# wavey-ai/soundkit

Hardware: AMD Instinct MI355X
Metric: AAC-LC 1024-sample frames/s (whole node) + xrealtime, batch=4096 48 kHz stereo (higher is better)
Workload: dtype f32 (synthesis f32; s16 between the kernels as in the reference; FIR: the 16-bit samples as 2 x f16 exactly, the f32 taps as 2 x f16 to 2^-24, f32 accumulate; 1.0e-7 rel. RMS vs f64)

## Files before the change

soundkit_amd/csrc/aac_synth.hip:

```cpp
#include "sk_device.h"

#define SK_SYNTH_LOAD(p) (*(p))
#define SK_SYNTH_STORE(v, p) (*(p) = (v))

namespace sk {

namespace {

typedef float f2 __attribute__((ext_vector_type(2)));
typedef float f4 __attribute__((ext_vector_type(4)));

#ifndef SK_SYNTH_BLOCK_WAVES
#define SK_SYNTH_BLOCK_WAVES 4
#endif
constexpr int kWavesPerBlock = SK_SYNTH_BLOCK_WAVES;
#ifndef SK_WAVES_PER_SIMD
#define SK_WAVES_PER_SIMD 3
#endif
#ifndef SK_PREFETCH_DEPTH
#define SK_PREFETCH_DEPTH 1
#endif
constexpr int kDepth = SK_PREFETCH_DEPTH;
constexpr int kWavesPerSimd = SK_WAVES_PER_SIMD;
constexpr int kExchange = 576;
// ... 495 lines not shown
    wave_sync();
    f2 o[16], d[16];
#pragma unroll
    for (int half = 0; half < 2; ++half) {
#pragma unroll
        for (int r = 0; r < 8; ++r) *reinterpret_cast<lds_f4 *>(stage + 2 * lane + 128 * r) = (f4){0.f, 0.f, 0.f, 0.f};
        wave_sync();
#pragma unroll
        for (int parity = 0; parity < 2; ++parity) {
#pragma unroll
            for (int w = parity; w < 8; w += 2)
#pragma unroll
                for (int m = 0; m < 4; ++m) {
                    const int base = 448 + 128 * w + 64 * m;
                    if ((base >> 10) != half) continue;
                    lds_f2 *at = stage + (base & 1023) + lane;
                    *at = *at + smp[w][m];
                }
            wave_sync();
        }
        if (half == 0) read_positions2(stage, lane, o);
        else read_positions2(stage, lane, d);
        wave_sync();
    }
    f2 pcm[16];
#pragma unroll
    for (int i = 0; i < 16; ++i) pcm[i] = o[i] + dly[i];
    write_positions2((lds_f2 *)ex, lane, pcm);
    write_positions2(stage, lane, d);
    wave_sync();
}

template <bool OUT16, bool WITH_SHORT>
__global__ __launch_bounds__(kWavesPerBlock * 64, 2) void k_aac_synth_pair(SynthArgs a) {
    constexpr bool LDS_WIN = !WITH_SHORT;
    __shared__ f4 lds[kWavesPerBlock][kPairExchange];
    __shared__ f4 win_tab[LDS_WIN ? 2048 : 1];
    __shared__ f2 stage_lds[WITH_SHORT ? kWavesPerBlock : 1][WITH_SHORT ? kStage : 2];
    __shared__ f2 tw_tab[512];
    __shared__ f2 t64_tab[64];
    __shared__ float short_win_tab[WITH_SHORT ? 512 : 2];
    __shared__ f2 short_tw_tab[WITH_SHORT ? 128 : 1];

    const int lane = threadIdx.x & 63;
    const int wave = __builtin_amdgcn_readfirstlane(threadIdx.x >> 6);
    for (int i = threadIdx.x; i < 512; i += kWavesPerBlock * 64) tw_tab[i] = reinterpret_cast<const f2 *>(a.t.tw_long)[i];
    if (threadIdx.x < 64) t64_tab[threadIdx.x] = reinterpret_cast<const f2 *>(a.t.w64)[((threadIdx.x >> 3) * (threadIdx.x & 7)) & 63];
    if (WITH_SHORT) {
        for (int i = threadIdx.x; i < 512; i += kWavesPerBlock * 64) short_win_tab[i] = a.t.win[4096 + i];
        if (threadIdx.x < 128)
            short_tw_tab[threadIdx.x] = threadIdx.x < 64 ? reinterpret_cast<const f2 *>(a.t.w64)[threadIdx.x] : reinterpret_cast<const f2 *>(a.t.tw_short)[threadIdx.x - 64];
    }
    if (LDS_WIN)
        for (int i = threadIdx.x; i < 2048; i += kWavesPerBlock * 64) win_tab[i] = reinterpret_cast<const f4 *>(a.t.win)[i < 1024 ? i : i + 128];
    __syncthreads();
    const lds_f *win_lds = (const lds_f *)win_tab;

    const uint32_t pair_id = blockIdx.x * kWavesPerBlock + wave;
    if (2 * pair_id + 1 >= a.n_tasks) return;
    lds_f4 *ex = (lds_f4 *)lds[wave];
    const lds_f2 *tw_lds = (const lds_f2 *)tw_tab;
    const lds_f2 *t64 = (const lds_f2 *)t64_tab;

    const SynthTask task_a = a.tasks[2 * pair_id], task_b = a.tasks[2 * pair_id + 1];
    const uint32_t count = __builtin_amdgcn_readfirstlane(task_a.count);
    if (count == 0) return;
    const uint32_t state_a = __builtin_amdgcn_readfirstlane(task_a.state), state_b = __builtin_amdgcn_readfirstlane(task_b.state);
    const const_entries ent_a = as_constant(a.entries + __builtin_amdgcn_readfirstlane(task_a.begin));
    const const_entries ent_b = as_constant(a.entries + __builtin_amdgcn_readfirstlane(task_b.begin));

    const int hi3 = lane >> 3, lo3 = lane & 7;
    const f2 base2 = reinterpret_cast<const f2 *>(a.t.w512)[hi3 * lo3];

    float *delay_a = a.delay + (size_t)state_a * 1024, *delay_b = a.delay + (size_t)state_b * 1024;
    int prev_a = __builtin_amdgcn_readfirstlane((int)a.prev_shape[state_a]);
    int prev_b = __builtin_amdgcn_readfirstlane((int)a.prev_shape[state_b]);
    float dly_a[16], dly_b[16];
    auto load_state = [&](const float *p, float (&d)[16]) {
#pragma unroll
        for (int r = 0; r < 2; ++r) {
            const int j = 4 * lane + 256 * r;
            const f4 f = *reinterpret_cast<const f4 *>(p + j);
            const f4 m = *reinterpret_cast<const f4 *>(p + 1020 - j);
            d[8 * r + 0] = f.x; d[8 * r + 1] = f.y; d[8 * r + 2] = f.z; d[8 * r + 3] = f.w;
            d[8 * r + 4] = m.x; d[8 * r + 5] = m.y; d[8 * r + 6] = m.z; d[8 * r + 7] = m.w;
        }
    };
    load_state(delay_a, dly_a);
    load_state(delay_b, dly_b);

    auto load_spectrum = [&](f2 (&xin)[8], const_entries entries, uint32_t e) {
        const float *src = a.coeffs + (size_t)__builtin_amdgcn_readfirstlane(entries[e].off1024) * 1024 + 2 * lane;
#pragma unroll
        for (int r = 0; r < 8; ++r) xin[r] = SK_SYNTH_LOAD(reinterpret_cast<const f2 *>(src + 128 * r));
    };
    struct Win {
        f4 w1f[2], w1m[2], w2f[2], w2m[2];
    };
    auto load_windows = [&](Win &w, int seq, int prev_shape, int shape) {
        const float *w1 = first_half_window(a.t.win, seq, prev_shape);
        const float *w2 = second_half_window(a.t.win, seq, shape);
#pragma unroll
        for (int r = 0; r < 2; ++r) {
            const int j = 4 * lane + 256 * r;
            w.w1f[r] = *reinterpret_cast<const f4 *>(w1 + j);
            w.w1m[r] = *reinterpret_cast<const f4 *>(w1 + 1020 - j);
            w.w2f[r] = *reinterpret_cast<const f4 *>(w2 + j);
            w.w2m[r] = *reinterpret_cast<const f4 *>(w2 + 1020 - j);
        }
    };
    auto emit = [&](int r, f2 F0, f2 F1, f2 M0, f2 M1, const Win &w, int w1_at, int w2_at, float (&dly)[16], float *out_ptr, int16_t *out16_ptr) {
        const int j = 4 * lane + 256 * r;
        f4 W1f, W1m, W2f, W2m;
        if constexpr (LDS_WIN) {
            W1f = *reinterpret_cast<const lds_f4 *>(win_lds + w1_at + j), W1m = *reinterpret_cast<const lds_f4 *>(win_lds + w1_at + 1020 - j);
            W2f = *reinterpret_cast<const lds_f4 *>(win_lds + w2_at + j), W2m = *reinterpret_cast<const lds_f4 *>(win_lds + w2_at + 1020 - j);
        } else {
            W1f = w.w1f[r], W1m = w.w1m[r], W2f = w.w2f[r], W2m = w.w2m[r];
        }
        f4 f, m;
        f.x = -F0.x * W1f.x + dly[8 * r + 0]; f.y = -M1.y * W1f.y + dly[8 * r + 1];
        f.z = -F1.x * W1f.z + dly[8 * r + 2]; f.w = -M0.y * W1f.w + dly[8 * r + 3];
        m.x = M0.y * W1m.x + dly[8 * r + 4]; m.y = F1.x * W1m.y + dly[8 * r + 5];
        m.z = M1.y * W1m.z + dly[8 * r + 6]; m.w = F0.x * W1m.w + dly[8 * r + 7];
        if (OUT16) {
            SK_SYNTH_STORE(pack4_s16(f), reinterpret_cast<u2 *>(out16_ptr + j));
            SK_SYNTH_STORE(pack4_s16(m), reinterpret_cast<u2 *>(out16_ptr + 1020 - j));
        } else {
            SK_SYNTH_STORE(f, reinterpret_cast<f4 *>(out_ptr + j));
            SK_SYNTH_STORE(m, reinterpret_cast<f4 *>(out_ptr + 1020 - j));
        }
        dly[8 * r + 0] = F0.y * W2f.x; dly[8 * r + 1] = M1.x * W2f.y;
        dly[8 * r + 2] = F1.y * W2f.z; dly[8 * r + 3] = M0.x * W2f.w;
        dly[8 * r + 4] = M0.x * W2m.x; dly[8 * r + 5] = F1.y * W2m.y;
        dly[8 * r + 6] = M1.x * W2m.z; dly[8 * r + 7] = F0.y * W2m.w;
    };

    lds_f2 *stage = (lds_f2 *)stage_lds[WITH_SHORT ? wave : 0];
    auto store_pcm = [&](const float (&pcm)[16], uint32_t off) __attribute__((always_inline)) {
#pragma unroll
        for (int r = 0; r < 2; ++r) {
            const int j = 4 * lane + 256 * r;
            const f4 f = (f4){pcm[8 * r + 0], pcm[8 * r + 1], pcm[8 * r + 2], pcm[8 * r + 3]};
            const f4 m = (f4){pcm[8 * r + 4], pcm[8 * r + 5], pcm[8 * r + 6], pcm[8 * r + 7]};
            if (OUT16) {
                SK_SYNTH_STORE(pack4_s16(f), reinterpret_cast<u2 *>(a.pcm16 + (size_t)off * 1024 + j));
                SK_SYNTH_STORE(pack4_s16(m), reinterpret_cast<u2 *>(a.pcm16 + (size_t)off * 1024 + 1020 - j));
            } else {
                SK_SYNTH_STORE(f, reinterpret_cast<f4 *>(a.pcm + (size_t)off * 1024 + j));
                SK_SYNTH_STORE(m, reinterpret_cast<f4 *>(a.pcm + (size_t)off * 1024 + 1020 - j));
            }
        }
    };

    f2 xa[8], xb[8];
    load_spectrum(xa, ent_a, 0);
    load_spectrum(xb, ent_b, 0);
    for (uint32_t e = 0; e < count; ++e) {
        const uint32_t off_a = __builtin_amdgcn_readfirstlane(ent_a[e].off1024), off_b = __builtin_amdgcn_readfirstlane(ent_b[e].off1024);
        const uint32_t win_a = __builtin_amdgcn_readfirstlane(ent_a[e].win), win_b = __builtin_amdgcn_readfirstlane(ent_b[e].win);
        const int shape_a = (win_a >> 2) & 1, shape_b = (win_b >> 2) & 1;
        if constexpr (WITH_SHORT) {
            if ((win_a & 3u) == 2u) {
// ... 51 lines not shown
            const f2 tx = splat(t.x), ty = splat(t.y);
            z[r] = {odd * ty - even * tx, odd * tx + even * ty};
        }
        Win wa, wb;
        int w1_a = 0, w2_a = 0, w1_b = 0, w2_b = 0;
        if constexpr (LDS_WIN) {
            const int seq_a = (int)(win_a & 3), seq_b = (int)(win_b & 3);
            w1_a = seq_a == 3 ? 6144 + 1024 * prev_a : 2048 * prev_a, w2_a = seq_a == 1 ? 4096 + 1024 * shape_a : 2048 * shape_a + 1024;
            w1_b = seq_b == 3 ? 6144 + 1024 * prev_b : 2048 * prev_b, w2_b = seq_b == 1 ? 4096 + 1024 * shape_b : 2048 * shape_b + 1024;
        } else {
            load_windows(wa, (int)(win_a & 3), prev_a, shape_a);
            load_windows(wb, (int)(win_b & 3), prev_b, shape_b);
        }
        {
            const uint32_t ahead = e + 1 < count ? e + 1 : count - 1;
            load_spectrum(xa, ent_a, ahead);
            load_spectrum(xb, ent_b, ahead);
        }
        fft512(z, ex, t64, base2, lane);
#pragma unroll
        for (int j = 0; j < 8; ++j) {
            const f2 t = tw_lds[lane + 64 * j];
            const f2 tx = splat(t.x), ty = splat(t.y);
            const c2 v = {fma2(tx, z[j].re, -(ty * -z[j].im)), fma2(tx, -z[j].im, ty * z[j].re)};
            ex[lane + 64 * j] = as_slot(v);
        }
        wave_sync();
        float *out_a = OUT16 ? nullptr : a.pcm + (size_t)off_a * 1024, *out_b = OUT16 ? nullptr : a.pcm + (size_t)off_b * 1024;
        int16_t *out16_a = OUT16 ? a.pcm16 + (size_t)off_a * 1024 : nullptr, *out16_b = OUT16 ? a.pcm16 + (size_t)off_b * 1024 : nullptr;
#pragma unroll
        for (int r = 0; r < 2; ++r) {
            const int q = 2 * lane + 128 * r;
            const f4 F0 = ex[256 + q], F1 = ex[257 + q], M0 = ex[254 - q], M1 = ex[255 - q];
            emit(r, (f2){F0.x, F0.z}, (f2){F1.x, F1.z}, (f2){M0.x, M0.z}, (f2){M1.x, M1.z}, wa, w1_a, w2_a, dly_a, out_a, out16_a);
            emit(r, (f2){F0.y, F0.w}, (f2){F1.y, F1.w}, (f2){M0.y, M0.w}, (f2){M1.y, M1.w}, wb, w1_b, w2_b, dly_b, out_b, out16_b);
        }
        wave_sync();
        prev_a = shape_a;
        prev_b = shape_b;
    }
    auto store_state = [&](float *p, const float (&d)[16]) {
#pragma unroll
        for (int r = 0; r < 2; ++r) {
            const int j = 4 * lane + 256 * r;
            *reinterpret_cast<f4 *>(p + j) = (f4){d[8 * r + 0], d[8 * r + 1], d[8 * r + 2], d[8 * r + 3]};
            *reinterpret_cast<f4 *>(p + 1020 - j) = (f4){d[8 * r + 4], d[8 * r + 5], d[8 * r + 6], d[8 * r + 7]};
        }
    };
    store_state(delay_a, dly_a);
    store_state(delay_b, dly_b);
    if (lane == 0) {
        a.prev_shape[state_a] = (uint8_t)prev_a;
        a.prev_shape[state_b] = (uint8_t)prev_b;
    }
}

constexpr int kTailRing = 2048;
constexpr int kTailDepth = 2;

__global__ __launch_bounds__(128, 2) void k_aac_tail(TailArgs ta) {
    const SynthArgs &a = ta.s;
    __shared__ f2 lds[2][kExchange];
    __shared__ f2 tw_tab[512];
    __shared__ f2 t64_tab[64];
    __shared__ __attribute__((aligned(16))) uint16_t ring_lds[2][2][kTailRing];
    __shared__ __attribute__((aligned(16))) uint32_t xchg[2][2][128];

    const int lane = threadIdx.x & 63;
    const int wave = __builtin_amdgcn_readfirstlane((int)(threadIdx.x >> 6));
    for (int i = threadIdx.x; i < 512; i += 128) tw_tab[i] = reinterpret_cast<const f2 *>(a.t.tw_long)[i];
    if (threadIdx.x < 64) t64_tab[threadIdx.x] = reinterpret_cast<const f2 *>(a.t.w64)[((threadIdx.x >> 3) * (threadIdx.x & 7)) & 63];
    for (int i = threadIdx.x; i < 2 * 2 * kTailRing / 8; i += 128) reinterpret_cast<sk_u32x4 *>(&ring_lds[0][0][0])[i] = (sk_u32x4){0u, 0u, 0u, 0u};
    __syncthreads();

    const uint32_t pair_id = blockIdx.x;
    lds_f2 *ex = (lds_f2 *)lds[wave];
    const lds_f2 *tw_lds = (const lds_f2 *)tw_tab;
    const lds_f2 *t64 = (const lds_f2 *)t64_tab;
    unsigned char *ring = reinterpret_cast<unsigned char *>(&ring_lds[wave][0][0]);

    const SynthTask task_v = a.tasks[2 * pair_id + (uint32_t)wave];
// ... 226 lines not shown
}

}

hipError_t launch_zero_spans(float *base, const uint32_t *ids, uint32_t n, uint32_t span_floats, hipStream_t s) {
    if (n == 0) return hipSuccess;
    if (span_floats % 4) return hipErrorInvalidValue;
    hipLaunchKernelGGL(k_zero_spans, dim3(n), dim3(256), 0, s, base, ids, span_floats);
    return hipGetLastError();
}

hipError_t launch_reset_streams(float *delay, uint8_t *shape, uint32_t *pns, const uint32_t *ids, uint32_t n, hipStream_t s) {
    if (n == 0) return hipSuccess;
    hipLaunchKernelGGL(k_reset_streams, dim3(n), dim3(256), 0, s, delay, shape, pns, ids);
    return hipGetLastError();
}

hipError_t launch_aac_synth(const SynthArgs &a, hipStream_t s) {
    if (a.n_tasks == 0) return hipSuccess;
    const uint32_t blocks = (a.n_tasks + kWavesPerBlock - 1) / kWavesPerBlock;
    if (a.only_long) {
        if (a.pcm16) hipLaunchKernelGGL((k_aac_synth<true, true>), dim3(blocks), dim3(kWavesPerBlock * 64), 0, s, a);
        else hipLaunchKernelGGL((k_aac_synth<false, true>), dim3(blocks), dim3(kWavesPerBlock * 64), 0, s, a);
    } else {
        if (a.pcm16) hipLaunchKernelGGL((k_aac_synth<true, false>), dim3(blocks), dim3(kWavesPerBlock * 64), 0, s, a);
        else hipLaunchKernelGGL((k_aac_synth<false, false>), dim3(blocks), dim3(kWavesPerBlock * 64), 0, s, a);
    }
    return hipGetLastError();
}

hipError_t launch_aac_synth_pairs(const SynthArgs &a, bool with_short, hipStream_t s) {
    if (a.n_tasks < 2) return hipSuccess;
    if (a.n_tasks & 1) return hipErrorInvalidValue;
    const uint32_t pairs = a.n_tasks / 2, blocks = (pairs + kWavesPerBlock - 1) / kWavesPerBlock;
    const dim3 grid(blocks), block(kWavesPerBlock * 64);
    if (with_short) {
        if (a.pcm16) hipLaunchKernelGGL((k_aac_synth_pair<true, true>), grid, block, 0, s, a);
        else hipLaunchKernelGGL((k_aac_synth_pair<false, true>), grid, block, 0, s, a);
    } else {
        if (a.pcm16) hipLaunchKernelGGL((k_aac_synth_pair<true, false>), grid, block, 0, s, a);
        else hipLaunchKernelGGL((k_aac_synth_pair<false, false>), grid, block, 0, s, a);
    }
    return hipGetLastError();
}

hipError_t launch_aac_tail(const TailArgs &ta, hipStream_t s) {
    if (ta.s.n_tasks < 2) return hipSuccess;
    if ((ta.s.n_tasks & 1) || !ta.afrag_f16 || !ta.out16 || ta.stream_stride == 0) return hipErrorInvalidValue;
    hipLaunchKernelGGL(k_aac_tail, dim3(ta.s.n_tasks / 2), dim3(128), 0, s, ta);
    return hipGetLastError();
}

hipError_t launch_frames_to_s16(const float *planar, int16_t *out, const FrameSpan *frames, uint32_t n, hipStream_t s) {
    if (n == 0) return hipSuccess;
    hipLaunchKernelGGL(k_frames_to_s16, dim3(n), dim3(256), 0, s, planar, out, frames, n);
    return hipGetLastError();
}

hipError_t launch_dequantize(const int16_t *q, const int16_t *sf, float *out, size_t n, const float *pow43,
                             const float *sftab, hipStream_t s) {
    if (n == 0) return hipSuccess;
    size_t blocks = (n + 255) / 256;
    if (blocks > 8192) blocks = 8192;
    hipLaunchKernelGGL(k_dequantize, dim3((unsigned)blocks), dim3(256), 0, s, q, sf, out, n, pow43, sftab);
    return hipGetLastError();
}

}
// ... 1 lines not shown
```

soundkit_amd/csrc/engine.cpp:

```cpp
#include "../../include/soundkit_amd.h"
#include "sk_abi.h"

#include <hip/hip_runtime.h>

#include <cmath>
#include <cstdio>
#include <chrono>
#include <cstdlib>
#include <cstring>
#include <algorithm>
#include <atomic>
#include <thread>
#include <map>
#include <mutex>
#include <new>
#include <string>
#include <unordered_map>
#include <vector>

#include "aac_entropy_tables.h"
#include "sk_device.h"

namespace {

// ... 136 lines not shown
        y[x] = val;
    }
    sum /= (float)factor;
    for (size_t p = 0; p < npoints; ++p) taps[p] = y[factor * p + (factor - 1)] / sum;
}

void make_sinc_table(double ratio, std::vector<float> &sincs) {
    const size_t npoints = 256, factor = 256, tot = npoints * factor;
    const float f_cutoff = ratio >= 1.0 ? 0.95f : 0.95f * (float)ratio;
    std::vector<float> y(tot);
    const float pi2 = 2.0f * kPiF, pi4 = 4.0f * kPiF, pi6 = 6.0f * kPiF, np_f = (float)tot;
    float sum = 0.0f;
    for (size_t x = 0; x < tot; ++x) {
        const float xf = (float)x;
        float w = 0.35875f - 0.48829f * std::cos(pi2 * xf / np_f) + 0.14128f * std::cos(pi4 * xf / np_f) -
                  0.01168f * std::cos(pi6 * xf / np_f);
        w = w * w;
        const float v = (xf - (float)(tot / 2)) * f_cutoff / (float)factor;
        const float sinc = v == 0.0f ? 1.0f : std::sin(v * kPiF) / (v * kPiF);
        const float val = w * sinc;
        sum += val;
        y[x] = val;
    }
    sum /= (float)factor;
    sincs.resize(tot);
    for (size_t p = 0; p < npoints; ++p)
        for (size_t n = 0; n < factor; ++n) sincs[(factor - n - 1) * npoints + p] = y[factor * p + n] / sum;
}

}

struct sk_engine {
    int device = -1;
    hipStream_t stream = nullptr;
    uint32_t max_streams = 0;
    std::mutex mu;
    std::string last_hip_error;

    std::vector<StreamInfo> streams;
    std::vector<uint32_t> free_ids;

    float *d_delay = nullptr;
    uint8_t *d_prev_shape = nullptr;
    float *d_rs = nullptr;
    float *d_mp3_tables = nullptr, *d_mp3_state = nullptr;
    bool mp3_window_set = false;
    uint8_t *d_mp3_rq = nullptr;
    uint16_t mp3_bands[sk::kMp3Rates][sk::kMp3BandRow] = {};
    bool mp3_bands_set[sk::kMp3Rates] = {};

    float *d_tables = nullptr;
    sk::SynthTables synth_tables{};
    float *d_pow43 = nullptr, *d_sftab = nullptr, *d_taps = nullptr, *d_zeros = nullptr;
    uint32_t *d_afrag16 = nullptr, *d_afrag_f16 = nullptr;
    std::vector<float> h_taps;
    std::vector<RatioTable> ratio_tables;

    DevBuf in_buf, out_buf, aux_buf, aux2_buf;
    DevBuf sinc_scratch;
    bool sinc_exact = false;
    DevBuf tick_pcm, tick_res, tick_out, tick_arena, tick_au, tick_side, tick_q, tick_mp3_in, tick_mp3_xr;
    uint32_t *d_pns = nullptr;
    void *d_ec_blob = nullptr;
    sk_ec::Tables ec_tables{};
    sk::EntropyArgs ec_args{};
    bool ec_ready = false;
    uint8_t *h_arena = nullptr;
    size_t h_arena_cap = 0;
    uint8_t *h_out = nullptr;
    size_t h_out_cap = 0;
    int32_t *h_status = nullptr;
    size_t h_status_cap = 0;
    std::vector<uint32_t> state_count, state_task;
    std::vector<uint32_t> pending_reset;
    std::vector<uint32_t> pending_rs_reset;
    uint32_t *d_rs_reset_ids = nullptr;
    uint32_t *d_reset_ids = nullptr;
    std::atomic<const char *> where{"idle"};
    double sync_timeout_s = 120.0;
    std::atomic<int> fail_after{0};

    int hip_fail(hipError_t e, const char *what) {
        last_hip_error = std::string(what) + ": " + hipGetErrorString(e);
        return e == hipErrorOutOfMemory ? SK_ERR_OOM : SK_ERR_HIP;
    }
};

struct sk_aac_plan {
    sk_engine *eng = nullptr;
    uint32_t n_tasks = 0, n_entries = 0, n_frames_ok = 0;
    uint64_t elements = 0;
    sk::SynthTask *d_tasks = nullptr;
    sk::SynthEntry *d_entries = nullptr;
    sk::FrameSpan *d_spans = nullptr;
    sk::SynthTask *d_pair_tasks = nullptr, *d_spair_tasks = nullptr, *d_long_tasks = nullptr, *d_walk_tasks = nullptr;
    uint32_t n_pair_tasks = 0, n_spair_tasks = 0, n_long_tasks = 0, n_walk_tasks = 0;
    uint32_t uniform_count = 0;
    uint32_t uniform_channels = 0;
};

#define SK_HIP(expr, what)                               \
    do {                                                  \
        hipError_t _e = (expr);                           \
        if (_e == hipSuccess && e->fail_after.load(std::memory_order_relaxed) > 0 && e->fail_after.fetch_sub(1) == 1) \
            _e = hipErrorLaunchFailure;  \
        if (_e != hipSuccess) return e->hip_fail(_e, what); \
    } while (0)

namespace {

std::mutex g_device_turn[16];
std::atomic<int> g_engines_on_device[16];
#if defined(SK_NO_DEVICE_TURNS) || !SK_PACKED_F32
constexpr int kTurnFrom = 1 << 30;
#else
constexpr int kTurnFrom = 1;
#endif

struct ComputeTurn {};
struct DeviceGuard {
    explicit DeviceGuard(int dev) { (void)hipGetDevice(&prev); if (prev != dev) (void)hipSetDevice(dev); want = dev; }
    explicit DeviceGuard(sk_engine *e);
    DeviceGuard(sk_engine *e, ComputeTurn);
    ~DeviceGuard() {
        if (turn.owns_lock()) {
            (void)hipStreamSynchronize(turn_stream);
            turn.unlock();
        }
        if (prev != want && prev >= 0) (void)hipSetDevice(prev);
// ... 196 lines not shown
    case SK_PIPE_CLOSED: return "Decode pipeline is closed";
    case SK_PIPE_CHUNK_TOO_LARGE: return "Input chunk exceeds the 4 MiB limit";
    case SK_AAC_ERR_EOF: return "unexpected end of AAC bitstream";
    case SK_AAC_ERR_INVALID_AOT: return "invalid AAC audio object type";
    case SK_AAC_ERR_UNSUPPORTED_AOT: return "unsupported AAC audio object type";
    case SK_AAC_ERR_UNSUPPORTED_SF_INDEX: return "unsupported AAC sampling frequency index";
    case SK_AAC_ERR_UNSUPPORTED_CHANNEL_CONFIG: return "unsupported AAC channel configuration";
    case SK_ERR_TIMEOUT: return "the device did not finish in time";
    case SK_ERR_INTERNAL: return "internal error (a C++ exception was caught at the ABI)";
    case SK_MP3_NEED_MORE: return "more MP3 input needed";
    case SK_MP3_NO_SYNC: return "not an MPEG audio frame header";
    case SK_MP3_UNSUPPORTED: return "unsupported MPEG audio layer or feature";
    case SK_MP3_INVALID: return "invalid MP3 side information";
    case SK_AAC_ERR_UNSUPPORTED_FEATURE: return "unsupported AAC feature";
    case SK_AAC_ERR_INVALID_CONFIG: return "invalid AAC config";
    case SK_AAC_ERR_INVALID_BITSTREAM: return "invalid AAC bitstream";
    default: return "unknown status";
    }
} catch (...) {
    (void)sk::abi_caught("sk_strerror");
    return sk::abi_message();
}

int sk_engine_create(int device, uint32_t max_streams, sk_engine **out) try {
    sk::abi_enter();
    if (!out || max_streams == 0) return SK_ERR_INVALID_ARG;
    *out = nullptr;
    int count = 0;
    if (hipGetDeviceCount(&count) != hipSuccess || device < 0 || device >= count) return SK_ERR_NO_DEVICE;
    sk_engine *e = new (std::nothrow) sk_engine();
    if (!e) return SK_ERR_OOM;
    e->device = device;
    e->max_streams = max_streams;
    g_engines_on_device[device & 15].fetch_add(1);
    DeviceGuard guard(device);
    int rc = SK_OK;
    do {
        hipError_t he = hipStreamCreateWithFlags(&e->stream, hipStreamNonBlocking);
        if (he != hipSuccess) { rc = e->hip_fail(he, "hipStreamCreate"); break; }
        const size_t states = (size_t)max_streams * 2;
        he = hipMalloc((void **)&e->d_delay, states * 1024 * sizeof(float));
        if (he != hipSuccess) { rc = e->hip_fail(he, "alloc delay"); break; }
        he = hipMalloc((void **)&e->d_prev_shape, states);
        if (he != hipSuccess) { rc = e->hip_fail(he, "alloc prev_shape"); break; }
        (void)hipMemset(e->d_delay, 0, states * 1024 * sizeof(float));
        (void)hipMemset(e->d_prev_shape, 0, states);
        he = hipMalloc((void **)&e->d_pns, (size_t)max_streams * sizeof(uint32_t));
        if (he != hipSuccess) { rc = e->hip_fail(he, "alloc pns state"); break; }
        rc = build_tables(e);
        if (rc != SK_OK) break;
        e->streams.resize(max_streams);
        e->free_ids.reserve(max_streams);
        for (uint32_t i = max_streams; i-- > 0;) e->free_ids.push_back(i);
        e->state_count.assign(states, 0);
        e->state_task.assign(states, 0);
    } while (0);
    if (rc != SK_OK) {
        sk_engine_destroy(e);
        return rc;
    }
    *out = e;
    return SK_OK;
} catch (...) {
    return sk::abi_caught("sk_engine_create");
}

// ... 190 lines not shown

int sk_stream_set_state(sk_engine *e, uint32_t id, const float *delay, const uint8_t *prev_shape) try {
    sk::abi_enter();
    if (!e || !delay || !prev_shape) return SK_ERR_INVALID_ARG;
    std::lock_guard<std::mutex> lock(e->mu);
    if (!stream_ok(e, id)) return SK_ERR_BAD_STREAM;
    const uint32_t ch = e->streams[id].channels;
    for (uint32_t c = 0; c < ch; ++c)
        if (prev_shape[c] > 1) return SK_ERR_INVALID_ARG;
    DeviceGuard guard(e);
    SK_HIP(hipMemcpyAsync(e->d_delay + (size_t)id * 2048, delay, ch * 1024 * sizeof(float), hipMemcpyHostToDevice,
                          e->stream), "set delay");
    SK_HIP(hipMemcpyAsync(e->d_prev_shape + (size_t)id * 2, prev_shape, ch, hipMemcpyHostToDevice, e->stream),
           "set shape");
    SK_HIP(hipStreamSynchronize(e->stream), "set state sync");
    return SK_OK;
} catch (...) {
    return sk::abi_caught("sk_stream_set_state");
}


void sk_aac_plan_destroy(sk_aac_plan *p) try {
    sk::abi_enter();
    if (!p) return;
    if (p->eng) {
        DeviceGuard guard(p->eng->device);
        if (p->d_tasks) (void)hipFree(p->d_tasks);
        if (p->d_entries) (void)hipFree(p->d_entries);
        if (p->d_spans) (void)hipFree(p->d_spans);
        if (p->d_walk_tasks) (void)hipFree(p->d_walk_tasks);
        if (p->d_long_tasks) (void)hipFree(p->d_long_tasks);
        if (p->d_pair_tasks) (void)hipFree(p->d_pair_tasks);
        if (p->d_spair_tasks) (void)hipFree(p->d_spair_tasks);
    }
    delete p;
} catch (...) {
    (void)sk::abi_caught("sk_aac_plan_destroy");
}

uint64_t sk_aac_plan_elements(const sk_aac_plan *p) try {
    sk::abi_enter();
    return p ? p->elements : 0;
} catch (...) {
    (void)sk::abi_caught("sk_aac_plan_elements");
    return 0;
}
uint32_t sk_aac_plan_frames_ok(const sk_aac_plan *p) try {
    sk::abi_enter();
    return p ? p->n_frames_ok : 0;
} catch (...) {
    (void)sk::abi_caught("sk_aac_plan_frames_ok");
    return 0;
}

}

namespace {

struct HostPlan {
    std::vector<sk::SynthTask> tasks;
    std::vector<sk::SynthEntry> entries;
    std::vector<sk::FrameSpan> spans;
    std::vector<uint32_t> entry_of;
    std::vector<sk::SynthTask> pair_tasks, spair_tasks, long_tasks, walk_tasks;
    uint32_t uniform_count = 0, uniform_channels = 0;
    uint32_t frames_ok = 0;
    uint64_t off1024 = 0;
};

int build_plan_host(sk_engine *e, const sk_aac_frame_desc *descs, uint32_t n, int32_t *status, HostPlan &hp, bool windows_known = true) {
    std::vector<uint32_t> touched;
    std::vector<uint8_t> ok(n, 0);
    uint32_t frames_ok = 0;
    for (uint32_t i = 0; i < n; ++i) {
        const sk_aac_frame_desc &d = descs[i];
        int32_t st = SK_FRAME_OK;
        if (!stream_ok(e, d.stream)) st = SK_FRAME_BAD_STREAM;
        else if (d.channels != e->streams[d.stream].channels) st = SK_FRAME_BAD_CHANNELS;
        else {
            for (uint32_t c = 0; c < d.channels; ++c)
                if (d.window_sequence[c] > 3 || d.window_shape[c] > 1) st = SK_FRAME_BAD_WINDOW;
        }
        if (status) status[i] = st;
        if (st != SK_FRAME_OK) continue;
        ok[i] = 1;
        ++frames_ok;
        for (uint32_t c = 0; c < d.channels; ++c) {
            const uint32_t state = d.stream * 2 + c;
            if (e->state_count[state]++ == 0) touched.push_back(state);
        }
    }
    std::vector<sk::SynthTask> &tasks = hp.tasks;
    tasks.assign(touched.size(), sk::SynthTask{});
    uint32_t n_entries = 0;
    for (size_t t = 0; t < touched.size(); ++t) {
        const uint32_t state = touched[t];
        tasks[t].state = state;
        tasks[t].begin = n_entries;
        tasks[t].count = 0;
        tasks[t].pad = 0;
        n_entries += e->state_count[state];
// ... 59 lines not shown
            uint64_t h = 0;
            for (uint32_t k = 0; windows_known && k < tasks[t].count; ++k)
                if ((entries[tasks[t].begin + k].win & 3u) == 2u) h = (h ^ (k + 1)) * 0x100000001b3ull + 0x9e3779b9u;
            keys[t] = Key{tasks[t].count, h};
            if (!windows_known || !use_pairs) continue;
            auto it = waiting.find(keys[t]);
            if (it == waiting.end()) {
                waiting.emplace(keys[t], t);
                continue;
            }
            const uint32_t u = it->second;
            bool same = true;
            for (uint32_t k = 0; same && keys[t].shorts && k < tasks[t].count; ++k)
                same = ((entries[tasks[t].begin + k].win & 3u) == 2u) == ((entries[tasks[u].begin + k].win & 3u) == 2u);
            if (!same) continue;
            partner[t] = (int32_t)u;
            partner[u] = (int32_t)t;
            waiting.erase(it);
        }
        for (uint32_t t = 0; t < tasks.size(); ++t) {
            const bool has_short = !windows_known || keys[t].shorts != 0;
            if (partner[t] >= 0) {
                if ((uint32_t)partner[t] < t) continue;
                std::vector<sk::SynthTask> &dst = has_short ? hp.spair_tasks : hp.pair_tasks;
                dst.push_back(tasks[t]);
                dst.push_back(tasks[(uint32_t)partner[t]]);
            } else if (has_short) {
                hp.walk_tasks.push_back(tasks[t]);
            } else {
                hp.long_tasks.push_back(tasks[t]);
            }
        }
    }
    return SK_OK;
}

}

extern "C" {

int sk_aac_plan_create(sk_engine *e, const sk_aac_frame_desc *descs, uint32_t n, int32_t *status, sk_aac_plan **out) try {
    sk::abi_enter();
    if (!e || !out || (n && !descs)) return SK_ERR_INVALID_ARG;
    *out = nullptr;
    std::lock_guard<std::mutex> lock(e->mu);
    DeviceGuard guard(e);
    HostPlan hp;
    int rc = build_plan_host(e, descs, n, status, hp);
    if (rc != SK_OK) return rc;

    sk_aac_plan *p = new (std::nothrow) sk_aac_plan();
    if (!p) return SK_ERR_OOM;
    p->eng = e;
    p->n_tasks = (uint32_t)hp.tasks.size();
    p->n_entries = (uint32_t)hp.entries.size();
    p->n_frames_ok = hp.frames_ok;
    p->elements = hp.off1024 * 1024;
    if (!hp.tasks.empty()) {
        hipError_t he = upload(&p->d_tasks, hp.tasks);
        if (he == hipSuccess) he = upload(&p->d_entries, hp.entries);
        if (he == hipSuccess) he = upload(&p->d_spans, hp.spans);
        if (he == hipSuccess && !hp.walk_tasks.empty()) he = upload(&p->d_walk_tasks, hp.walk_tasks);
        if (he == hipSuccess && !hp.long_tasks.empty()) he = upload(&p->d_long_tasks, hp.long_tasks);
        if (he == hipSuccess && !hp.pair_tasks.empty()) he = upload(&p->d_pair_tasks, hp.pair_tasks);
        if (he == hipSuccess && !hp.spair_tasks.empty()) he = upload(&p->d_spair_tasks, hp.spair_tasks);
        p->n_walk_tasks = (uint32_t)hp.walk_tasks.size();
        p->n_long_tasks = (uint32_t)hp.long_tasks.size();
        p->n_pair_tasks = (uint32_t)hp.pair_tasks.size();
        p->n_spair_tasks = (uint32_t)hp.spair_tasks.size();
        p->uniform_count = hp.uniform_count;
        p->uniform_channels = hp.uniform_channels;
        if (he != hipSuccess) {
            sk_aac_plan_destroy(p);
            return e->hip_fail(he, "upload plan");
        }
    }
    *out = p;
    return SK_OK;
} catch (...) {
    return sk::abi_caught("sk_aac_plan_create");
}

static int run_plan(sk_engine *e, const sk_aac_plan *p, const float *d_coeffs, float *d_pcm, int16_t *d_pcm16 = nullptr) {
    sk::SynthArgs a{};
    a.coeffs = d_coeffs;
    a.pcm = d_pcm;
    a.pcm16 = d_pcm16;
    a.delay = e->d_delay;
    a.prev_shape = e->d_prev_shape;
    a.entries = p->d_entries;
    a.t = e->synth_tables;
    a.only_long = 1;
    a.tasks = p->d_pair_tasks;
    a.n_tasks = p->n_pair_tasks;
    SK_HIP(sk::launch_aac_synth_pairs(a, false, e->stream), "launch aac synth (two channels per wave)");
    a.tasks = p->d_spair_tasks;
    a.n_tasks = p->n_spair_tasks;
    SK_HIP(sk::launch_aac_synth_pairs(a, true, e->stream), "launch aac synth (two channels per wave, eight-short arm)");
    a.tasks = p->d_long_tasks;
    a.n_tasks = p->n_long_tasks;
    SK_HIP(sk::launch_aac_synth(a, e->stream), "launch aac synth (one channel per wave, no EightShort)");
    a.tasks = p->d_walk_tasks;
    a.n_tasks = p->n_walk_tasks;
    a.only_long = 0;
    SK_HIP(sk::launch_aac_synth(a, e->stream), "launch aac synth");
    return SK_OK;
}

int sk_aac_plan_run_f32_dev(sk_engine *e, const sk_aac_plan *p, const float *d_coeffs, float *d_pcm) try {
    sk::abi_enter();
    if (!e || !p || p->eng != e) return SK_ERR_INVALID_ARG;
    if (p->n_tasks == 0) return SK_OK;
    if (!d_coeffs || !d_pcm) return SK_ERR_INVALID_ARG;
    std::lock_guard<std::mutex> lock(e->mu);
    DeviceGuard guard(e, ComputeTurn{});
    return run_plan(e, p, d_coeffs, d_pcm);
} catch (...) {
    return sk::abi_caught("sk_aac_plan_run_f32_dev");
}

int sk_aac_plan_run_s16_planar_dev(sk_engine *e, const sk_aac_plan *p, const float *d_coeffs, int16_t *d_pcm16) try {
    sk::abi_enter();
    if (!e || !p || p->eng != e) return SK_ERR_INVALID_ARG;
    if (p->n_tasks == 0) return SK_OK;
    if (!d_coeffs || !d_pcm16 || ((uintptr_t)d_pcm16 & 7)) return SK_ERR_INVALID_ARG;
    std::lock_guard<std::mutex> lock(e->mu);
    DeviceGuard guard(e, ComputeTurn{});
// ... 2082 lines not shown
                SK_HIP(sk::launch_aac_entropy_parallel(ea, e->stream), "launch entropy decode");
            }
            if (e->h_status_cap < n_frames) {
                if (e->h_status) (void)hipHostFree(e->h_status);
                e->h_status = nullptr;
                e->h_status_cap = 0;
                const size_t want = (size_t)n_frames + (size_t)n_frames / 2 + 1024;
                SK_HIP(hipHostMalloc((void **)&e->h_status, want * sizeof(int32_t), hipHostMallocDefault), "alloc pinned status");
                e->h_status_cap = want;
            }
            SK_HIP(hipMemcpyAsync(e->h_status, d_status, (size_t)n_frames * sizeof(int32_t), hipMemcpyDeviceToHost, e->stream),
                   "D2H entropy status");
            status_pinned = true;
        }
        if (probe) {
            std::vector<sk::SynthEntry> got(hp.entries.size());
            SK_HIP(hipMemcpyAsync(got.data(), a.entries, got.size() * sizeof(sk::SynthEntry), hipMemcpyDeviceToHost, e->stream),
                   "D2H entropy window fields");
            SK_HIP(hipMemcpyAsync(probe->spectra, e->in_buf.p, elems * 4, hipMemcpyDeviceToHost, e->stream), "D2H entropy spectra");
            SK_HIP(hipStreamSynchronize(e->stream), "entropy sync");
            if (status_pinned) std::memcpy(status.data(), e->h_status, (size_t)n_frames * sizeof(int32_t));
            for (uint32_t k = 0; k < n_frames; ++k) {
                probe->status[k] = status[k];
                probe->descs[k] = descs[k];
                for (uint32_t c = 0; c < descs[k].channels; ++c) {
                    const uint32_t win = got[hp.entry_of[(size_t)k * 2 + c]].win;
                    probe->descs[k].window_sequence[c] = (uint8_t)(win & 3u);
                    probe->descs[k].window_shape[c] = (uint8_t)((win >> 2) & 1u);
                }
            }
            return SK_OK;
        }
        a.only_long = 1;
        if (!hp.pair_tasks.empty()) {
            SK_HIP(aux.put(hp.pair_tasks, e->stream, &a.tasks), "upload tick pair tasks");
            a.n_tasks = (uint32_t)hp.pair_tasks.size();
            SK_HIP(sk::launch_aac_synth_pairs(a, false, e->stream), "launch tick synth (two channels per wave)");
        }
        if (!hp.spair_tasks.empty()) {
            SK_HIP(aux.put(hp.spair_tasks, e->stream, &a.tasks), "upload tick pair tasks with EightShort frames");
            a.n_tasks = (uint32_t)hp.spair_tasks.size();
            SK_HIP(sk::launch_aac_synth_pairs(a, true, e->stream), "launch tick synth (two channels per wave, eight-short arm)");
        }
        if (!hp.long_tasks.empty()) {
            SK_HIP(aux.put(hp.long_tasks, e->stream, &a.tasks), "upload tick tasks without EightShort frames");
            a.n_tasks = (uint32_t)hp.long_tasks.size();
            SK_HIP(sk::launch_aac_synth(a, e->stream), "launch tick synth (one channel per wave, no EightShort)");
        }
        if (!hp.walk_tasks.empty()) {
            SK_HIP(aux.put(hp.walk_tasks, e->stream, &a.tasks), "upload tick walk tasks");
            a.n_tasks = (uint32_t)hp.walk_tasks.size();
            a.only_long = 0;
            SK_HIP(sk::launch_aac_synth(a, e->stream), "launch tick synth");
        }
        if (au_mode || q_mode) {
            const TClock::time_point q0 = TClock::now();
            t_au[0] = std::chrono::duration<double, std::milli>(q0 - t_mark).count();
            rc = wait_stream(e, "tick: waiting for the front-end kernels and the synthesis (mid-tick status read-back)");
            if (rc != SK_OK) return rc;
            if (status_pinned) std::memcpy(status.data(), e->h_status, (size_t)n_frames * sizeof(int32_t));
            e->where.store("tick: resampler rounds, pack");
            t_au[1] = std::chrono::duration<double, std::milli>(TClock::now() - q0).count();
            for (uint32_t i = 0; i < n_streams; ++i) {
                if (tc[i].mp3) continue;
                tc[i].good = ts[i].n_frames;
                tc[i].bad_status = 0;
                for (uint32_t f = 0; f < ts[i].n_frames; ++f)
                    if (status[tc[i].first + f] != 0) {
                        tc[i].good = f;
// ... 375 lines not shown
```

soundkit_amd/csrc/sk_device.h:

```cpp
#pragma once
#include <hip/hip_runtime.h>
#include <stdint.h>

#include "../../include/soundkit_amd.h"

namespace sk {

struct SynthEntry {
    uint32_t off1024;
    uint32_t win;
};

struct SynthTask {
    uint32_t state;
    uint32_t begin;
    uint32_t count;
    uint32_t pad;
};

struct SynthTables {
    const float2 *tw_long;
    const float2 *tw_short;
    const float2 *w64;
    const float2 *w512;
    const float *win;
};

struct SynthArgs {
    const float *coeffs;
    float *pcm;
    int16_t *pcm16;
    float *delay;
    uint8_t *prev_shape;
    const SynthTask *tasks;
    const SynthEntry *entries;
    uint32_t n_tasks;
    uint32_t only_long;
    SynthTables t;
};

struct FrameSpan {
    uint32_t off1024;
    uint32_t channels;
};

hipError_t launch_aac_synth(const SynthArgs &a, hipStream_t s);
struct TailArgs {
    SynthArgs s;
    const uint32_t *afrag_f16;
    int16_t *out16;
    size_t out_stride;
// ... 282 lines not shown
```

Measured before the change: 265.2 million.

## Split long pair synthesis tasks into frame ranges with warm-up frames

```diff
diff --git a/soundkit_amd/csrc/aac_synth.hip b/soundkit_amd/csrc/aac_synth.hip
--- a/soundkit_amd/csrc/aac_synth.hip
+++ b/soundkit_amd/csrc/aac_synth.hip
@@ -551,11 +551,12 @@
 }
 
 template <bool OUT16, bool WITH_SHORT>
-__global__ __launch_bounds__(kWavesPerBlock * 64, 2) void k_aac_synth_pair(SynthArgs a) {
+__global__ __launch_bounds__((WITH_SHORT ? kWavesPerBlock : (int)kPairRangeWaves) * 64, WITH_SHORT ? 2 : 3) void k_aac_synth_pair(SynthArgs a) {
     constexpr bool LDS_WIN = !WITH_SHORT;
-    __shared__ f4 lds[kWavesPerBlock][kPairExchange];
+    constexpr int kWaves = WITH_SHORT ? kWavesPerBlock : (int)kPairRangeWaves;
+    __shared__ f4 lds[kWaves][kPairExchange];
     __shared__ f4 win_tab[LDS_WIN ? 2048 : 1];
-    __shared__ f2 stage_lds[WITH_SHORT ? kWavesPerBlock : 1][WITH_SHORT ? kStage : 2];
+    __shared__ f2 stage_lds[WITH_SHORT ? kWaves : 1][WITH_SHORT ? kStage : 2];
     __shared__ f2 tw_tab[512];
     __shared__ f2 t64_tab[64];
     __shared__ float short_win_tab[WITH_SHORT ? 512 : 2];
@@ -563,37 +564,18 @@
 
     const int lane = threadIdx.x & 63;
     const int wave = __builtin_amdgcn_readfirstlane(threadIdx.x >> 6);
-    for (int i = threadIdx.x; i < 512; i += kWavesPerBlock * 64) tw_tab[i] = reinterpret_cast<const f2 *>(a.t.tw_long)[i];
-    if (threadIdx.x < 64) t64_tab[threadIdx.x] = reinterpret_cast<const f2 *>(a.t.w64)[((threadIdx.x >> 3) * (threadIdx.x & 7)) & 63];
-    if (WITH_SHORT) {
-        for (int i = threadIdx.x; i < 512; i += kWavesPerBlock * 64) short_win_tab[i] = a.t.win[4096 + i];
-        if (threadIdx.x < 128)
-            short_tw_tab[threadIdx.x] = threadIdx.x < 64 ? reinterpret_cast<const f2 *>(a.t.w64)[threadIdx.x] : reinterpret_cast<const f2 *>(a.t.tw_short)[threadIdx.x - 64];
-    }
-    if (LDS_WIN)
-        for (int i = threadIdx.x; i < 2048; i += kWavesPerBlock * 64) win_tab[i] = reinterpret_cast<const f4 *>(a.t.win)[i < 1024 ? i : i + 128];
-    __syncthreads();
-    const lds_f *win_lds = (const lds_f *)win_tab;
-
-    const uint32_t pair_id = blockIdx.x * kWavesPerBlock + wave;
-    if (2 * pair_id + 1 >= a.n_tasks) return;
-    lds_f4 *ex = (lds_f4 *)lds[wave];
-    const lds_f2 *tw_lds = (const lds_f2 *)tw_tab;
-    const lds_f2 *t64 = (const lds_f2 *)t64_tab;
-
-    const SynthTask task_a = a.tasks[2 * pair_id], task_b = a.tasks[2 * pair_id + 1];
+    const uint32_t pair_id = blockIdx.x * kWaves + wave;
+    const bool active = 2 * pair_id + 1 < a.n_tasks;
+    SynthTask task_a{}, task_b{};
+    if (active) {
+        task_a = a.tasks[2 * pair_id];
+        task_b = a.tasks[2 * pair_id + 1];
+    }
     const uint32_t count = __builtin_amdgcn_readfirstlane(task_a.count);
-    if (count == 0) return;
+    const uint32_t flags = WITH_SHORT ? 0u : __builtin_amdgcn_readfirstlane(task_a.pad);
     const uint32_t state_a = __builtin_amdgcn_readfirstlane(task_a.state), state_b = __builtin_amdgcn_readfirstlane(task_b.state);
-    const const_entries ent_a = as_constant(a.entries + __builtin_amdgcn_readfirstlane(task_a.begin));
-    const const_entries ent_b = as_constant(a.entries + __builtin_amdgcn_readfirstlane(task_b.begin));
-
-    const int hi3 = lane >> 3, lo3 = lane & 7;
-    const f2 base2 = reinterpret_cast<const f2 *>(a.t.w512)[hi3 * lo3];
-
     float *delay_a = a.delay + (size_t)state_a * 1024, *delay_b = a.delay + (size_t)state_b * 1024;
-    int prev_a = __builtin_amdgcn_readfirstlane((int)a.prev_shape[state_a]);
-    int prev_b = __builtin_amdgcn_readfirstlane((int)a.prev_shape[state_b]);
+    int prev_a = 0, prev_b = 0;
     float dly_a[16], dly_b[16];
     auto load_state = [&](const float *p, float (&d)[16]) {
 #pragma unroll
@@ -605,8 +587,38 @@
             d[8 * r + 4] = m.x; d[8 * r + 5] = m.y; d[8 * r + 6] = m.z; d[8 * r + 7] = m.w;
         }
     };
-    load_state(delay_a, dly_a);
-    load_state(delay_b, dly_b);
+    if (active && count != 0 && !(flags & kRangeWarm)) {
+        prev_a = __builtin_amdgcn_readfirstlane((int)a.prev_shape[state_a]);
+        prev_b = __builtin_amdgcn_readfirstlane((int)a.prev_shape[state_b]);
+        load_state(delay_a, dly_a);
+        load_state(delay_b, dly_b);
+    } else {
+#pragma unroll
+        for (int i = 0; i < 16; ++i) dly_a[i] = dly_b[i] = 0.f;
+    }
+    for (int i = threadIdx.x; i < 512; i += kWaves * 64) tw_tab[i] = reinterpret_cast<const f2 *>(a.t.tw_long)[i];
+    if (threadIdx.x < 64) t64_tab[threadIdx.x] = reinterpret_cast<const f2 *>(a.t.w64)[((threadIdx.x >> 3) * (threadIdx.x & 7)) & 63];
+    if (WITH_SHORT) {
+        for (int i = threadIdx.x; i < 512; i += kWaves * 64) short_win_tab[i] = a.t.win[4096 + i];
+        if (threadIdx.x < 128)
+            short_tw_tab[threadIdx.x] = threadIdx.x < 64 ? reinterpret_cast<const f2 *>(a.t.w64)[threadIdx.x] : reinterpret_cast<const f2 *>(a.t.tw_short)[threadIdx.x - 64];
+    }
+    if (LDS_WIN)
+        for (int i = threadIdx.x; i < 2048; i += kWaves * 64) win_tab[i] = reinterpret_cast<const f4 *>(a.t.win)[i < 1024 ? i : i + 128];
+    __syncthreads();
+    const lds_f *win_lds = (const lds_f *)win_tab;
+
+    if (!active || count == 0) return;
+    lds_f4 *ex = (lds_f4 *)lds[wave];
+    const lds_f2 *tw_lds = (const lds_f2 *)tw_tab;
+    const lds_f2 *t64 = (const lds_f2 *)t64_tab;
+
+    const const_entries ent_a = as_constant(a.entries + __builtin_amdgcn_readfirstlane(task_a.begin));
+    const const_entries ent_b = as_constant(a.entries + __builtin_amdgcn_readfirstlane(task_b.begin));
+
+    const int hi3 = lane >> 3, lo3 = lane & 7;
+    const f2 base2 = reinterpret_cast<const f2 *>(a.t.w512)[hi3 * lo3];
+    const uint32_t first_out = (flags & kRangeWarm) ? 1u : 0u;
 
     auto load_spectrum = [&](f2 (&xin)[8], const_entries entries, uint32_t e) {
         const float *src = a.coeffs + (size_t)__builtin_amdgcn_readfirstlane(entries[e].off1024) * 1024 + 2 * lane;
@@ -628,7 +640,8 @@
             w.w2m[r] = *reinterpret_cast<const f4 *>(w2 + 1020 - j);
         }
     };
-    auto emit = [&](int r, f2 F0, f2 F1, f2 M0, f2 M1, const Win &w, int w1_at, int w2_at, float (&dly)[16], float *out_ptr, int16_t *out16_ptr) {
+    auto emit = [&](int r, f2 F0, f2 F1, f2 M0, f2 M1, const Win &w, int w1_at, int w2_at, float (&dly)[16], float *out_ptr, int16_t *out16_ptr,
+                    bool out) {
         const int j = 4 * lane + 256 * r;
         f4 W1f, W1m, W2f, W2m;
         if constexpr (LDS_WIN) {
@@ -637,17 +650,19 @@
         } else {
             W1f = w.w1f[r], W1m = w.w1m[r], W2f = w.w2f[r], W2m = w.w2m[r];
         }
-        f4 f, m;
-        f.x = -F0.x * W1f.x + dly[8 * r + 0]; f.y = -M1.y * W1f.y + dly[8 * r + 1];
-        f.z = -F1.x * W1f.z + dly[8 * r + 2]; f.w = -M0.y * W1f.w + dly[8 * r + 3];
-        m.x = M0.y * W1m.x + dly[8 * r + 4]; m.y = F1.x * W1m.y + dly[8 * r + 5];
-        m.z = M1.y * W1m.z + dly[8 * r + 6]; m.w = F0.x * W1m.w + dly[8 * r + 7];
-        if (OUT16) {
-            SK_SYNTH_STORE(pack4_s16(f), reinterpret_cast<u2 *>(out16_ptr + j));
-            SK_SYNTH_STORE(pack4_s16(m), reinterpret_cast<u2 *>(out16_ptr + 1020 - j));
-        } else {
-            SK_SYNTH_STORE(f, reinterpret_cast<f4 *>(out_ptr + j));
-            SK_SYNTH_STORE(m, reinterpret_cast<f4 *>(out_ptr + 1020 - j));
+        if (out) {
+            f4 f, m;
+            f.x = -F0.x * W1f.x + dly[8 * r + 0]; f.y = -M1.y * W1f.y + dly[8 * r + 1];
+            f.z = -F1.x * W1f.z + dly[8 * r + 2]; f.w = -M0.y * W1f.w + dly[8 * r + 3];
+            m.x = M0.y * W1m.x + dly[8 * r + 4]; m.y = F1.x * W1m.y + dly[8 * r + 5];
+            m.z = M1.y * W1m.z + dly[8 * r + 6]; m.w = F0.x * W1m.w + dly[8 * r + 7];
+            if (OUT16) {
+                SK_SYNTH_STORE(pack4_s16(f), reinterpret_cast<u2 *>(out16_ptr + j));
+                SK_SYNTH_STORE(pack4_s16(m), reinterpret_cast<u2 *>(out16_ptr + 1020 - j));
+            } else {
+                SK_SYNTH_STORE(f, reinterpret_cast<f4 *>(out_ptr + j));
+                SK_SYNTH_STORE(m, reinterpret_cast<f4 *>(out_ptr + 1020 - j));
+            }
         }
         dly[8 * r + 0] = F0.y * W2f.x; dly[8 * r + 1] = M1.x * W2f.y;
         dly[8 * r + 2] = F1.y * W2f.z; dly[8 * r + 3] = M0.x * W2f.w;
@@ -765,8 +780,8 @@
         for (int r = 0; r < 2; ++r) {
             const int q = 2 * lane + 128 * r;
             const f4 F0 = ex[256 + q], F1 = ex[257 + q], M0 = ex[254 - q], M1 = ex[255 - q];
-            emit(r, (f2){F0.x, F0.z}, (f2){F1.x, F1.z}, (f2){M0.x, M0.z}, (f2){M1.x, M1.z}, wa, w1_a, w2_a, dly_a, out_a, out16_a);
-            emit(r, (f2){F0.y, F0.w}, (f2){F1.y, F1.w}, (f2){M0.y, M0.w}, (f2){M1.y, M1.w}, wb, w1_b, w2_b, dly_b, out_b, out16_b);
+            emit(r, (f2){F0.x, F0.z}, (f2){F1.x, F1.z}, (f2){M0.x, M0.z}, (f2){M1.x, M1.z}, wa, w1_a, w2_a, dly_a, out_a, out16_a, e >= first_out);
+            emit(r, (f2){F0.y, F0.w}, (f2){F1.y, F1.w}, (f2){M0.y, M0.w}, (f2){M1.y, M1.w}, wb, w1_b, w2_b, dly_b, out_b, out16_b, e >= first_out);
         }
         wave_sync();
         prev_a = shape_a;
@@ -780,6 +795,7 @@
             *reinterpret_cast<f4 *>(p + 1020 - j) = (f4){d[8 * r + 4], d[8 * r + 5], d[8 * r + 6], d[8 * r + 7]};
         }
     };
+    if (flags & kRangeKeep) return;
     store_state(delay_a, dly_a);
     store_state(delay_b, dly_b);
     if (lane == 0) {
@@ -1072,8 +1088,9 @@
 hipError_t launch_aac_synth_pairs(const SynthArgs &a, bool with_short, hipStream_t s) {
     if (a.n_tasks < 2) return hipSuccess;
     if (a.n_tasks & 1) return hipErrorInvalidValue;
-    const uint32_t pairs = a.n_tasks / 2, blocks = (pairs + kWavesPerBlock - 1) / kWavesPerBlock;
-    const dim3 grid(blocks), block(kWavesPerBlock * 64);
+    const uint32_t waves = with_short ? kWavesPerBlock : kPairRangeWaves;
+    const uint32_t pairs = a.n_tasks / 2, blocks = (pairs + waves - 1) / waves;
+    const dim3 grid(blocks), block(waves * 64);
     if (with_short) {
         if (a.pcm16) hipLaunchKernelGGL((k_aac_synth_pair<true, true>), grid, block, 0, s, a);
         else hipLaunchKernelGGL((k_aac_synth_pair<false, true>), grid, block, 0, s, a);
diff --git a/soundkit_amd/csrc/engine.cpp b/soundkit_amd/csrc/engine.cpp
--- a/soundkit_amd/csrc/engine.cpp
+++ b/soundkit_amd/csrc/engine.cpp
@@ -192,6 +192,7 @@
 
 struct sk_engine {
     int device = -1;
+    uint32_t cus = 0;
     hipStream_t stream = nullptr;
     uint32_t max_streams = 0;
     std::mutex mu;
@@ -255,6 +256,8 @@
     sk::FrameSpan *d_spans = nullptr;
     sk::SynthTask *d_pair_tasks = nullptr, *d_spair_tasks = nullptr, *d_long_tasks = nullptr, *d_walk_tasks = nullptr;
     uint32_t n_pair_tasks = 0, n_spair_tasks = 0, n_long_tasks = 0, n_walk_tasks = 0;
+    sk::SynthTask *d_range_tasks = nullptr;
+    uint32_t n_range_tasks = 0;
     uint32_t uniform_count = 0;
     uint32_t uniform_channels = 0;
 };
@@ -517,6 +520,10 @@
     if (!e) return SK_ERR_OOM;
     e->device = device;
     e->max_streams = max_streams;
+    {
+        int cus = 0;
+        if (hipDeviceGetAttribute(&cus, hipDeviceAttributeMultiprocessorCount, device) == hipSuccess && cus > 0) e->cus = (uint32_t)cus;
+    }
     g_engines_on_device[device & 15].fetch_add(1);
     DeviceGuard guard(device);
     int rc = SK_OK;
@@ -773,6 +780,7 @@
         if (p->d_long_tasks) (void)hipFree(p->d_long_tasks);
         if (p->d_pair_tasks) (void)hipFree(p->d_pair_tasks);
         if (p->d_spair_tasks) (void)hipFree(p->d_spair_tasks);
+        if (p->d_range_tasks) (void)hipFree(p->d_range_tasks);
     }
     delete p;
 } catch (...) {
@@ -804,10 +812,50 @@
     std::vector<sk::FrameSpan> spans;
     std::vector<uint32_t> entry_of;
     std::vector<sk::SynthTask> pair_tasks, spair_tasks, long_tasks, walk_tasks;
+    std::vector<sk::SynthTask> range_tasks;
     uint32_t uniform_count = 0, uniform_channels = 0;
     uint32_t frames_ok = 0;
     uint64_t off1024 = 0;
 };
+
+void plan_pair_ranges(const std::vector<sk::SynthTask> &pairs, uint32_t cus, std::vector<sk::SynthTask> &out) {
+    out.clear();
+    const uint64_t n_pairs = pairs.size() / 2;
+    if (n_pairs == 0) return;
+    uint32_t longest = 0;
+    for (const sk::SynthTask &t : pairs) longest = std::max(longest, t.count);
+    uint32_t best = 1;
+    uint64_t best_cost = ~0ull;
+    for (uint32_t r : {1u, 2u, 3u, 4u, 6u, 12u}) {
+        if (cus == 0 && r > 1) break;
+        const uint64_t per_group = sk::kPairRangeWaves / r, groups = (n_pairs + per_group - 1) / per_group;
+        const uint64_t rounds = cus ? (groups + cus - 1) / cus : 1;
+        const uint64_t cost = rounds * ((longest + r - 1) / r + (r > 1 ? 1 : 0));
+        if (cost < best_cost) best_cost = cost, best = r;
+    }
+    out.reserve(n_pairs * 2 * best);
+    for (uint64_t p = 0; p < n_pairs; ++p) {
+        const sk::SynthTask &ta = pairs[2 * p], &tb = pairs[2 * p + 1];
+        const uint32_t c = ta.count, used = std::min(best, c);
+        uint32_t at = 0;
+        for (uint32_t i = 0; i < best; ++i) {
+            const uint32_t n = i < used ? c / used + (i < c % used ? 1 : 0) : 0;
+            sk::SynthTask ra = ta, rb = tb;
+            if (n == 0) {
+                ra.count = rb.count = 0;
+                ra.pad = rb.pad = 0;
+            } else {
+                const uint32_t warm = at > 0 ? 1 : 0;
+                ra.begin = ta.begin + at - warm, rb.begin = tb.begin + at - warm;
+                ra.count = rb.count = n + warm;
+                ra.pad = rb.pad = (warm ? sk::kRangeWarm : 0u) | (at + n < c ? sk::kRangeKeep : 0u);
+            }
+            out.push_back(ra);
+            out.push_back(rb);
+            at += n;
+        }
+    }
+}
 
 int build_plan_host(sk_engine *e, const sk_aac_frame_desc *descs, uint32_t n, int32_t *status, HostPlan &hp, bool windows_known = true) {
     std::vector<uint32_t> touched;
@@ -933,6 +981,7 @@
             }
         }
     }
+    plan_pair_ranges(hp.pair_tasks, e->cus, hp.range_tasks);
     return SK_OK;
 }
 
@@ -965,10 +1014,12 @@
         if (he == hipSuccess && !hp.long_tasks.empty()) he = upload(&p->d_long_tasks, hp.long_tasks);
         if (he == hipSuccess && !hp.pair_tasks.empty()) he = upload(&p->d_pair_tasks, hp.pair_tasks);
         if (he == hipSuccess && !hp.spair_tasks.empty()) he = upload(&p->d_spair_tasks, hp.spair_tasks);
+        if (he == hipSuccess && !hp.range_tasks.empty()) he = upload(&p->d_range_tasks, hp.range_tasks);
         p->n_walk_tasks = (uint32_t)hp.walk_tasks.size();
         p->n_long_tasks = (uint32_t)hp.long_tasks.size();
         p->n_pair_tasks = (uint32_t)hp.pair_tasks.size();
         p->n_spair_tasks = (uint32_t)hp.spair_tasks.size();
+        p->n_range_tasks = (uint32_t)hp.range_tasks.size();
         p->uniform_count = hp.uniform_count;
         p->uniform_channels = hp.uniform_channels;
         if (he != hipSuccess) {
@@ -992,8 +1043,8 @@
     a.entries = p->d_entries;
     a.t = e->synth_tables;
     a.only_long = 1;
-    a.tasks = p->d_pair_tasks;
-    a.n_tasks = p->n_pair_tasks;
+    a.tasks = p->d_range_tasks;
+    a.n_tasks = p->n_range_tasks;
     SK_HIP(sk::launch_aac_synth_pairs(a, false, e->stream), "launch aac synth (two channels per wave)");
     a.tasks = p->d_spair_tasks;
     a.n_tasks = p->n_spair_tasks;
@@ -3142,9 +3193,9 @@
             return SK_OK;
         }
         a.only_long = 1;
-        if (!hp.pair_tasks.empty()) {
-            SK_HIP(aux.put(hp.pair_tasks, e->stream, &a.tasks), "upload tick pair tasks");
-            a.n_tasks = (uint32_t)hp.pair_tasks.size();
+        if (!hp.range_tasks.empty()) {
+            SK_HIP(aux.put(hp.range_tasks, e->stream, &a.tasks), "upload tick pair tasks");
+            a.n_tasks = (uint32_t)hp.range_tasks.size();
             SK_HIP(sk::launch_aac_synth_pairs(a, false, e->stream), "launch tick synth (two channels per wave)");
         }
         if (!hp.spair_tasks.empty()) {
diff --git a/soundkit_amd/csrc/sk_device.h b/soundkit_amd/csrc/sk_device.h
--- a/soundkit_amd/csrc/sk_device.h
+++ b/soundkit_amd/csrc/sk_device.h
@@ -17,6 +17,10 @@
     uint32_t count;
     uint32_t pad;
 };
+
+constexpr uint32_t kRangeWarm = 1;
+constexpr uint32_t kRangeKeep = 2;
+constexpr uint32_t kPairRangeWaves = 12;
 
 struct SynthTables {
     const float2 *tw_long;
```

New measurement: 263.3 million, median of 4. No clear change (-0.7%).
